# jkk-research/urban_road_filter

Hardware: AMD Instinct MI355X
Metric: scans/sec (64-ring x 2048-column cloud) (higher is better)
Workload: dtype f32+f64; 1 GPU; cfg3: batch of 1024 independent 64x2048 street sweeps per GPU, all three detectors + blind_spots, reference default parameters with ROI x,y widened to +-200 m, inputs resident in HBM (SoA x/y/z); scans_per_gpu=1024

## Files before the change

urban_road_filter_amd/csrc/urf_api.hip:

```cpp
#include <hip/hip_runtime.h>

#include <cmath>
#include <cstdio>
#include <cstdlib>
#include <cstring>
#include <ctime>
#include <string>
#include <vector>
#if defined(__SSE2__)
#include <emmintrin.h>
#include <xmmintrin.h>
#endif

#include "urf.h"
#ifdef URF_ENABLE_TEST_HOOKS
#include "urf_test_hooks.h"
#endif
#include "urf_internal.hpp"
#include "urf_kernels.hpp"
#include "urf_front.hpp"

#define URF_ASYNC_SLOTS 4
static_assert(URF_ASYNC_SLOTS == URF_MAX_IN_FLIGHT, "include/urf.h documents the number of sweeps in flight");

template <class T, bool Host = false>
struct lazy_buf {
    T* p = nullptr;
    size_t cap = 0;
    lazy_buf() = default;
    lazy_buf(const lazy_buf&) = delete;
    lazy_buf& operator=(const lazy_buf&) = delete;
    ~lazy_buf() { release(); }
    void release()
    {
        if (p)
            (void)(Host ? hipHostFree(p) : hipFree(p));
        p = nullptr;
        cap = 0;
    }
};

#define URF_SCRATCH_SCANS(X)                                                                                                     \
    X(rx, sstride) X(ry, sstride) X(rz, sstride) X(rec, sstride)                                                                 \
    X(sr, sstride) X(sz, sstride) X(sslot, sstride) X(ssrt16, sstride) X(ssrt, sstride) X(wsg, sstride)                          \
    X(big_r, sstride) X(big_z, sstride) X(big_i, sstride)                                                                        \
    X(tile_roi, max_tiles) X(roi_bits, max_tiles * (URF_TILE / 64)) X(troff, max_tiles * (URF_MAX_CHANNELS + 1))                 \
    X(tsoff, max_tiles * (URF_MAX_SECTORS + 1)) X(tmaxs, max_tiles * URF_MAX_CHANNELS)                                           \
    X(rpre, URF_MAX_CHANNELS * (max_tiles + 1)) X(rstart, URF_MAX_CHANNELS * max_tiles)                                          \
    X(angle, URF_MAX_CHANNELS) X(ring_thr, URF_MAX_CHANNELS * 4) X(ring_lut, URF_LUT_CELLS) X(ring_cnt, URF_MAX_CHANNELS)        \
    X(ring_off, URF_MAX_CHANNELS + 1)                                                                                            \
    X(sec_cnt, URF_MAX_SECTORS) X(sec_run, URF_MAX_SECTORS) X(sec_off, URF_MAX_SECTORS + 1) X(star_hit, URF_MAX_SECTORS)         \
    X(star_first, URF_MAX_SECTORS) X(star_list_mid, URF_MAX_SECTORS) X(star_list_big, URF_MAX_SECTORS)                           \
    X(star_list_runs, URF_MAX_SECTORS) X(tie_list, URF_MAX_SECTORS) X(tie_post, URF_MAX_SECTORS)                                 \
    X(table_upto, 1) X(table_redo, 1) X(redo_list, 1) X(table_cause, 1)                                                          \
    X(nan_mask, 4) X(nan_list, 2 * URF_MAX_CHANNELS) X(vis, URF_MAX_CHANNELS)                                                    \
    X(maxdist, URF_MAX_CHANNELS) X(quad, 4)                                                                                      \
    X(curb_cnt, URF_MAX_CHANNELS) X(curb_az, URF_MAX_CHANNELS * URF_CURB_LIST)                                                   \
    X(sufmin, URF_MAX_CHANNELS * URF_DEG_CELLS) X(premax, URF_MAX_CHANNELS * URF_DEG_CELLS)                                      \
    X(stop_f, URF_DEG_CELLS) X(stop_b, URF_DEG_CELLS)                                                                            \
    X(win, URF_MAX_CHANNELS * URF_DEG_CELLS)                                                                                     \
    X(info, 1)                                                                                                                   \
    X(front_ok, 1) X(front_pres, max_tiles * 64) X(front_maxs, max_tiles * 64) X(front_lane_ring, 64)                            \
    X(front_ring_lane, URF_MAX_CHANNELS) X(front_cand, front_cand_cap) X(front_all, front_cand_cap) X(front_ncand, 1)             \
    X(front_list, 1) X(front_st, URF_FRONT_ST_WORDS)
#define URF_SCRATCH_SLOTS(X) X(star_count, 8) X(ring_hint, 1)
#define URF_SCRATCH_CAPTURE(X) X(valpha, sstride) X(seckey, sstride) X(ringkey, sstride) X(rd2, sstride) X(caz, sstride)
#define URF_SCRATCH_ROW_MAJOR(X) X(tx, sstride) X(ty, sstride) X(tz, sstride) X(rows_v, 64) X(rows_ok, 1)
enum urf_scratch_group { URF_SCR_ALWAYS, URF_SCR_CAPTURE, URF_SCR_ROW_MAJOR };

struct __attribute__((visibility("hidden"))) urf_policy {
    uint32_t* flags = nullptr;
    uint64_t epoch = 1;
    bool speculate = true, use_hint = true;
    bool slot_lists = false, slot_nan = false, slot_ties = false;
    int front_mode = 1;
    uint32_t front_tpb = 0;
    bool want_ring_sorted = false;
    bool front_direct = false, front_off = false;
    bool front_rows = false, rows_oom = false, rows_used = false;
    uint32_t rows_probation = 0;

    template <class T>
    void set(T& field, T value)
    {
        if (field != value) {
            field = value;
            epoch++;
        }
    }
    void forget_front()
    {
        set(front_direct, false);
        set(front_off, false);
        flags[URF_FLAG_FRONT_HANDED_BACK] = flags[URF_FLAG_FRONT_ALL_HANDED_BACK] = 0;
    }
    int fold(urf_ctx* c, hipStream_t st);
    void probation_sweep() { lapse(front_rows); }
    void probation_batch(const urf_kargs& a) { lapse(a.front && front_mode != 2 && a.n_scans < URF_FRONT_MIN_SCANS); }
    void lapse(bool counts)
    {
        if (counts && !rows_used && rows_probation && --rows_probation == 0)
            epoch++;
    }
    bool on_redo(int status)
    {
        switch (status) {
        case URF_STATUS_REDO_TABLE: set(speculate, false); return true;
        case URF_STATUS_REDO_HINT: set(use_hint, false); return true;
        case URF_STATUS_REDO_LISTS: set(slot_lists, true); return true;
        case URF_STATUS_REDO_NAN: set(slot_nan, true); return true;
        case URF_STATUS_REDO_TIES: set(slot_ties, true); return true;
        }
        return false;
    }
    void plan(urf_kargs& a, const urf_dev_params& dp, bool slot, bool general_only) const
    {
        a.table_lookahead = speculate ? URF_TABLE_LOOKAHEAD : 0u;
        a.table_hint = (speculate && use_hint) ? 1u : 0u;
        a.optimistic = slot ? ((speculate ? URF_OPT_NO_REPAIR : 0u) | (slot_lists ? 0u : URF_OPT_NO_LISTS) | (slot_nan ? 0u : URF_OPT_NO_NAN) |
                               (slot_ties ? 0u : URF_OPT_NO_TIES)) : 0u;
        const unsigned L = (unsigned)dp.p.channels;
        const bool lasers = L == 64u || L == 32u || L == 16u;
        a.front_lsh = L == 16u ? 4u : (L == 32u ? 5u : 6u);
        const bool shape = front_mode != 0 && !front_off && !general_only && !want_ring_sorted && a.capture == 0 &&
                           lasers && dp.p.curbPoints == 5 && a.tiles <= URF_FRONT_MAX_TILES;
        const bool small_ok = front_rows && (rows_used || rows_probation > 0) && (L == 64u || front_mode == 2);
        a.front = (shape && (slot ? small_ok : (front_mode == 2 || small_ok || a.n_scans >= (L == 64u ? URF_FRONT_MIN_SCANS : (L == 32u ? URF_FRONT_MIN_SCANS_32 : URF_FRONT_MIN_SCANS_16))))) ? 1u : 0u;
        a.front_sight = (shape && !a.front && !front_rows && !rows_oom && (L == 64u || front_mode == 2)) ? 1u : 0u;
        a.front_tpb = front_tpb ? front_tpb : (a.n_scans >= URF_FRONT_TPB_SCANS ? URF_FRONT_TPB_LARGE : (a.n_scans >= 16u ? URF_FRONT_TPB_SMALL : 1u));
        a.front_lists = (a.front && !front_direct && !slot) ? 1u : 0u;
        a.front_rows = (a.front && front_rows) ? 1u : 0u;
    }
};

enum urf_last_kind { URF_LAST_NONE, URF_LAST_SOA, URF_LAST_PC2, URF_LAST_SWEEP };
struct urf_last_call {
    int kind = URF_LAST_NONE;
    uint32_t scans = 0;
    urf_kargs a;
    urf_dev_params dp;
    uint32_t row = 0;
    uint64_t gen = 0;
};

struct urf_ctx {
    int device = 0;
    uint32_t max_points = 0, max_batch = 0;
    uint32_t max_tiles = 0;
    uint32_t sstride = 0;
    uint32_t debug_flags = 0;
    unsigned n_cus = 256;
    hipStream_t own_stream = nullptr;
    hipStream_t stream = nullptr;
    urf_params params;
    urf_dev_params dp;
    urf_kargs k;
    std::vector<void*> allocs;
    lazy_buf<float> sx, sy, sz;
    struct slot_t {
        lazy_buf<uint8_t, true> h_in;
        lazy_buf<uint8_t> d_raw;
        lazy_buf<uint8_t, true> h_labels;
        lazy_buf<uint8_t> d_labels;
        lazy_buf<urf_scan_info, true> h_info;
        hipEvent_t ev_done = nullptr;
        hipGraph_t graph = nullptr;
        hipGraphExec_t exec = nullptr;
        uint64_t key[3] = { 0, 0, 0 };
        urf_kargs cap_a;
        urf_dev_params cap_dp;
        bool pending = false, used = false;
        uint64_t gen = 0;
        uint32_t n_points = 0, ticket = 0;
        uint32_t point_step = 0, off_x = 0, off_y = 0, off_z = 0;
        bool planes = false;
    } slots[URF_ASYNC_SLOTS];
    bool streams_made = false;
    urf_policy pol;
    uint32_t n_rerun = 0;
    hipStream_t row_stream[URF_ASYNC_SLOTS] = { nullptr, nullptr, nullptr, nullptr };
    hipEvent_t ev_main = nullptr;
    uint64_t main_seq = 1;
    uint64_t row_seen[URF_ASYNC_SLOTS] = { 0, 0, 0, 0 };
    uint64_t row_gen[URF_ASYNC_SLOTS] = { 0, 0, 0, 0 };
    uint32_t next_ticket = 0;
    lazy_buf<unsigned long long> ord_keys;
    lazy_buf<uint32_t> ord_pos;
    lazy_buf<uint32_t> ord_cls;
    lazy_buf<uint32_t> ord_lists;
    lazy_buf<float> mk_d;
    lazy_buf<uint32_t> mk_pos;
    lazy_buf<uint8_t> mk_red;
    lazy_buf<float> mk_out;
    lazy_buf<int32_t> mk_ghost;
    uint32_t* compact_cnt = nullptr;
    lazy_buf<urf_u32x4> cl_tiles;
    lazy_buf<uint32_t> cl_lists;
    float* d_newY = nullptr;
    urf_beam* d_beams = nullptr;
    uint32_t beams_cap = 0;
    int capture = 0;
    bool timing = false;
    std::vector<std::vector<hipEvent_t>> timing_events;
    size_t timing_used = 0;
    uint32_t* offsets_copy = nullptr;
    hipStream_t side_stream = nullptr;
    hipEvent_t ev_fork = nullptr, ev_join = nullptr;
    urf_last_call last;
    std::string last_error;
    double ht[8] = { 0, 0, 0, 0, 0, 0, 0, 0 };
    bool ht_on = false;
};

#define URF_HIP(ctx, call)                                                              \
    do {                                                                                \
        hipError_t e_ = (call);                                                         \
        if (e_ != hipSuccess) {                                                         \
            (ctx)->last_error = std::string(#call) + ": " + hipGetErrorString(e_);      \
            return e_ == hipErrorOutOfMemory ? URF_ERR_OOM : URF_ERR_HIP;               \
        }                                                                               \
    } while (0)

template <class T>
static int dev_alloc(urf_ctx* c, T** p, size_t count)
{
    void* v = nullptr;
    URF_HIP(c, hipMalloc(&v, (count ? count : 1) * sizeof(T)));
    c->allocs.push_back(v);
    *p = (T*)v;
    return URF_OK;
}

template <class T, bool Host>
static int grow(urf_ctx* c, lazy_buf<T, Host>& b, size_t count, hipStream_t st = nullptr)
{
    if (count <= b.cap)
        return URF_OK;
    if (st)
        URF_HIP(c, hipStreamSynchronize(st));
    b.release();
    void* v = nullptr;
    URF_HIP(c, Host ? hipHostMalloc(&v, count * sizeof(T), hipHostMallocDefault) : hipMalloc(&v, count * sizeof(T)));
    b.p = (T*)v;
    b.cap = count;
    return URF_OK;
}
// ... 123 lines not shown
extern "C" int urf_create(urf_ctx** out, int device_id, uint32_t max_points, uint32_t max_batch)
{
    if (!out || max_points == 0 || max_batch == 0)
        return URF_ERR_INVALID_ARG;
    *out = nullptr;
    const unsigned long long max_tiles = ((unsigned long long)max_points + URF_TILE - 1) / URF_TILE;
    const unsigned long long sstride = max_tiles * URF_TILE + URF_SCAN_PAD;
    if (max_tiles > URF_MAX_TILES || sstride * max_batch >= (1ull << 32))
        return URF_ERR_CAPACITY;
    int ndev = 0;
    if (hipGetDeviceCount(&ndev) != hipSuccess || ndev <= 0 || device_id < 0 || device_id >= ndev)
        return URF_ERR_NO_DEVICE;
    urf_ctx* c = new urf_ctx();
    c->device = device_id;
    c->max_points = max_points;
    c->max_batch = max_batch;
    c->max_tiles = (uint32_t)max_tiles;
    c->sstride = (uint32_t)sstride;
    int rc = URF_OK;
    auto fail = [&](int code) {
        urf_destroy(c);
        return code;
    };
    if (hipSetDevice(device_id) != hipSuccess)
        return fail(URF_ERR_NO_DEVICE);
    if (hipStreamCreateWithFlags(&c->own_stream, hipStreamNonBlocking) != hipSuccess)
        return fail(URF_ERR_HIP);
    c->stream = c->own_stream;
    {
        hipDeviceProp_t prop;
        if (hipGetDeviceProperties(&prop, device_id) == hipSuccess && prop.multiProcessorCount > 0)
            c->n_cus = (unsigned)prop.multiProcessorCount;
    }
    urf_default_params(&c->params);
    std::memset(&c->k, 0, sizeof(c->k));
    std::memset(&c->last.a, 0, sizeof(c->last.a));
    urf_kargs& k = c->k;
    k.front_cand_cap = max_points / 8 > 4096 ? max_points / 8 : 4096;
    if ((rc = scratch_alloc(c, URF_SCR_ALWAYS)) != URF_OK || (rc = dev_alloc(c, &c->offsets_copy, (size_t)max_batch + 1)) != URF_OK ||
        (rc = dev_alloc(c, &c->compact_cnt, (size_t)max_batch * c->max_tiles * 4)) != URF_OK ||
        (rc = dev_alloc(c, &c->d_newY, (size_t)max_points)) != URF_OK || (rc = dev_alloc(c, &c->d_beams, (size_t)URF_MAX_SECTORS)) != URF_OK)
        return fail(rc);
    {
        urf_wu* tab = nullptr;
        const size_t nt = (size_t)max_points + 32;
        if ((rc = dev_alloc(c, &tab, nt)) != URF_OK)
            return fail(rc);
        hipLaunchKernelGGL(k_walk_table, dim3((unsigned)((nt + 255) / 256)), dim3(256), 0, c->stream, tab, (unsigned)nt);
        k.walk_tab = tab;
    }
    k.sstride = c->sstride;
    if (const char* e = std::getenv("URF_FRONT_TPB"))
        c->pol.front_tpb = (uint32_t)std::atoi(e) > 0 ? (uint32_t)std::atoi(e) : c->pol.front_tpb;
    {
        void* hp = nullptr;
        if (hipHostMalloc(&hp, URF_FLAG_WORDS * sizeof(uint32_t), hipHostMallocMapped) != hipSuccess)
            return fail(URF_ERR_HIP);
        c->pol.flags = (uint32_t*)hp;
        std::memset(hp, 0, URF_FLAG_WORDS * sizeof(uint32_t));
        if (hipMemset(k.ring_hint, 0, URF_ASYNC_SLOTS * sizeof(uint32_t)) != hipSuccess)
            return fail(URF_ERR_HIP);
        void* dp_ = nullptr;
        if (hipHostGetDevicePointer(&dp_, hp, 0) != hipSuccess)
            return fail(URF_ERR_HIP);
        k.flags = (uint32_t*)dp_;
    }
    {
        std::vector<float> newY(max_points);
        newY[0] = 0.0f;
        for (uint32_t j = 1; j < max_points; j++)
            newY[j] = (float)((double)newY[j - 1] + 0.0100);
        if (hipMemcpy(c->d_newY, newY.data(), newY.size() * sizeof(float), hipMemcpyHostToDevice) != hipSuccess)
            return fail(URF_ERR_HIP);
    }
    k.newY = c->d_newY;
    k.beams = c->d_beams;
    if ((rc = upload_params(c)) != URF_OK)
        return fail(rc);
    *out = c;
    return URF_OK;
}

extern "C" int urf_destroy(urf_ctx* c)
{
    if (!c)
        return URF_ERR_INVALID_ARG;
    (void)hipSetDevice(c->device);
    if (c->own_stream)
        (void)hipStreamSynchronize(c->own_stream);
    if (c->side_stream) {
        (void)hipStreamSynchronize(c->side_stream);
        (void)hipStreamDestroy(c->side_stream);
        (void)hipEventDestroy(c->ev_fork);
        (void)hipEventDestroy(c->ev_join);
    }
    for (hipStream_t st : c->row_stream)
        if (st)
            (void)hipStreamSynchronize(st);
    for (auto& set : c->timing_events)
        for (hipEvent_t e : set)
            (void)hipEventDestroy(e);
    for (void* p : c->allocs)
        (void)hipFree(p);
    if (c->pol.flags)
        (void)hipHostFree(c->pol.flags);
    for (auto& sl : c->slots) {
// ... 189 lines not shown
static int order_after_slots(urf_ctx* c)
{
    for (auto& sl : c->slots)
        if (sl.pending && sl.ev_done)
            URF_HIP(c, hipStreamWaitEvent(c->stream, sl.ev_done, 0));
    c->main_seq++;
    return URF_OK;
}
static int order_row_after_main(urf_ctx* c, uint32_t row, hipStream_t st)
{
    if (st == c->stream || c->row_seen[row] == c->main_seq)
        return URF_OK;
    if (!c->ev_main)
        URF_HIP(c, hipEventCreateWithFlags(&c->ev_main, hipEventDisableTiming));
    URF_HIP(c, hipEventRecord(c->ev_main, c->stream));
    URF_HIP(c, hipStreamWaitEvent(st, c->ev_main, 0));
    c->row_seen[row] = c->main_seq;
    return URF_OK;
}

struct urf_call {
    const float *x, *y, *z;
    const uint32_t* offsets;
    uint32_t n_per_scan, max_len, n_scans;
    uint8_t* labels;
    urf_scan_info* info;
    uint32_t row = 0;
    hipStream_t stream = nullptr;
    const urf_dev_params* dp = nullptr;
    int capture = -1;
    bool general_only = false;
};

static bool side_fork(urf_ctx* c, hipStream_t st)
{
    if (!c->side_stream) {
        hipStream_t s = nullptr;
        hipEvent_t f = nullptr, j = nullptr;
        if (hipStreamCreateWithFlags(&s, hipStreamNonBlocking) == hipSuccess && hipEventCreateWithFlags(&f, hipEventDisableTiming) == hipSuccess &&
            hipEventCreateWithFlags(&j, hipEventDisableTiming) == hipSuccess) {
            c->side_stream = s;
            c->ev_fork = f;
            c->ev_join = j;
        } else {
            if (f)
                (void)hipEventDestroy(f);
            if (s)
                (void)hipStreamDestroy(s);
        }
    }
    return c->side_stream && hipEventRecord(c->ev_fork, st) == hipSuccess && hipStreamWaitEvent(c->side_stream, c->ev_fork, 0) == hipSuccess;
}

static int run_pipeline(urf_ctx* c, const urf_call& call, urf_kargs& a_out, urf_dev_params& dp_out)
{
    if (!call.x || !call.y || !call.z || !call.labels)
        return URF_ERR_INVALID_ARG;
    const uint32_t n_scans = call.n_scans;
    if (n_scans == 0)
        return URF_OK;
    if (call.row + n_scans > c->max_batch || call.max_len > c->max_points)
        return URF_ERR_CAPACITY;
    URF_HIP(c, hipSetDevice(c->device));
    const bool slot = call.stream != nullptr;
    hipStream_t st = slot ? call.stream : c->stream;
    if (!slot) {
        int rc = order_after_slots(c);
        if (rc == URF_OK)
            rc = c->pol.fold(c, st);
        if (rc != URF_OK)
            return rc;
    }
    urf_kargs a = kargs_row(c, call.row);
    a.x = call.x;
    a.y = call.y;
    a.z = call.z;
    a.offsets = nullptr;
    if (call.offsets) {
        if (call.offsets != c->offsets_copy)
            URF_HIP(c, hipMemcpyAsync(c->offsets_copy, call.offsets, ((size_t)n_scans + 1) * sizeof(uint32_t), hipMemcpyDeviceToDevice, st));
        a.offsets = c->offsets_copy;
    }
    a.n_per_scan = call.n_per_scan;
    a.n_scans = n_scans;
    a.max_len = call.max_len;
    a.tiles = (call.max_len + URF_TILE - 1) / URF_TILE;
    if (a.tiles == 0)
        a.tiles = 1;
    a.sstride = c->sstride;
    a.capture = (uint32_t)(call.capture >= 0 ? call.capture : c->capture);
    a.labels = call.labels;
    if (a.capture != 1) {
        a.rd2 = nullptr;
        a.caz = nullptr;
    }
    const urf_dev_params dp = call.dp ? *call.dp : c->dp;
    const unsigned C = (unsigned)dp.p.channels, K = (unsigned)dp.p.sectors;
    const bool star = dp.p.star_shaped_method != 0;
    const dim3 g_tiles(a.tiles, n_scans), g_scan(n_scans);
    c->pol.plan(a, dp, slot, call.general_only);
    if (!slot)
        c->pol.probation_batch(a);

    std::vector<hipEvent_t>* ev = nullptr;
    if (c->timing) {
        if (c->timing_used == c->timing_events.size()) {
            c->timing_events.emplace_back(URF_NUM_KERNELS + 1);
            for (hipEvent_t& e : c->timing_events.back())
                URF_HIP(c, hipEventCreate(&e));
        }
        ev = &c->timing_events[c->timing_used++];
    }
    int stage = 0;
    auto mark = [&]() {
        if (ev)
            (void)hipEventRecord((*ev)[stage], st);
        stage++;
    };
    mark();
    if (a.front_rows)
        hipLaunchKernelGGL(k_rows_probe, g_scan, dim3(256), 0, st, a, dp);
    hipLaunchKernelGGL(k_ring_table, g_scan, dim3(URF_TABLE_THREADS), 0, st, a, dp);
    mark();
    if (a.front_rows)
        hipLaunchKernelGGL(k_transpose, g_tiles, dim3(256), 0, st, a);
    if (a.front) {
        const dim3 g_front((a.tiles + a.front_tpb - 1) / a.front_tpb, n_scans);
        if (a.front_lsh == 6u)
            hipLaunchKernelGGL(k_front, g_front, dim3(64), 0, st, a, dp);
        else if (a.front_lsh == 5u)
            hipLaunchKernelGGL(k_front32, g_front, dim3(64), 0, st, a, dp);
        else
            hipLaunchKernelGGL(k_front16, g_front, dim3(64), 0, st, a, dp);
    }
    if (a.front_lists) {
        hipLaunchKernelGGL(k_table_repair, g_scan, dim3(URF_TABLE_THREADS), 0, st, a, dp, 1u);
        hipLaunchKernelGGL(k_split_list, dim3(c->n_cus * 2), dim3(URF_TILE_THREADS), urf_split_lds_bytes(C, K, star), st, a, dp);
    } else {
        hipLaunchKernelGGL(k_split, g_tiles, dim3(URF_TILE_THREADS), urf_split_lds_bytes(C, K, star), st, a, dp);
    }
    if ((a.table_lookahead || a.front_rows) && !(a.optimistic & URF_OPT_NO_REPAIR)) {
        hipLaunchKernelGGL(k_table_repair, g_scan, dim3(URF_TABLE_THREADS), 0, st, a, dp, 0u);
        hipLaunchKernelGGL(k_split_repair, dim3(c->n_cus), dim3(URF_TILE_THREADS), urf_split_lds_bytes(C, K, star), st, a, dp);
    }
    mark();
    bool side = false, part1 = false;
    const size_t finish_lds = (size_t)a.tiles * 384 + 2 * URF_FINISH_CHUNK * sizeof(urf_u2);
    if (a.front && !ev && !slot && side_fork(c, st)) {
        hipLaunchKernelGGL(k_front_finish, g_scan, dim3(URF_FINISH_THREADS), finish_lds, c->side_stream, a, dp, 1u);
        part1 = true;
        side = hipEventRecord(c->ev_join, c->side_stream) == hipSuccess;
        if (!side)
            (void)hipStreamSynchronize(c->side_stream);
    }
    hipLaunchKernelGGL(k_index, g_scan, dim3(256), 0, st, a, dp);
    mark();
    const unsigned tie_grid = K * n_scans < c->n_cus * 4u ? K * n_scans : c->n_cus * 4u;
    const unsigned tie_grid_small = K * n_scans < c->n_cus * 16u ? K * n_scans : c->n_cus * 16u;
    if (star) {
        const dim3 g_sec(K, n_scans);
        hipLaunchKernelGGL(k_star_sort_small, g_sec, dim3(URF_STAR_THREADS), 0, st, a, dp);
        if (!(a.optimistic & URF_OPT_NO_LISTS)) {
            hipLaunchKernelGGL(k_star_sort_mid, dim3(c->n_cus * (URF_MID_WAVES * 256 / URF_STAR_MID_THREADS)), dim3(URF_STAR_MID_THREADS), 0, st,
                               a, dp);
            hipLaunchKernelGGL(k_star_sort_big, dim3(c->n_cus * 2), dim3(256), 0, st, a, dp);
            hipLaunchKernelGGL(k_star_sort_runs, dim3(c->n_cus * 20), dim3(URF_STAR_THREADS), 0, st, a, dp);
        }
        if (!(a.optimistic & URF_OPT_NO_TIES)) {
            hipLaunchKernelGGL((k_star_ties<false, URF_TIE_SMALL>), dim3(tie_grid_small), dim3(64), 0, st, a, dp);
            hipLaunchKernelGGL((k_star_ties<false, URF_TIE_CAP>), dim3(tie_grid), dim3(64), 0, st, a, dp);
        }
    }
    mark();
    if (star) {
        if (n_scans <= URF_WALK_FEW_SCANS)
            hipLaunchKernelGGL(k_star_walk_few, dim3((K + 63) / 64, n_scans), dim3(URF_WALK_FEW_THREADS), 0, st, a, dp);
        else
            hipLaunchKernelGGL(k_star_walk, dim3((K + 63) / 64, n_scans), dim3(64), 0, st, a, dp);
        if (!(a.optimistic & URF_OPT_NO_TIES)) {
            hipLaunchKernelGGL((k_star_ties<true, URF_TIE_SMALL>), dim3(tie_grid_small), dim3(64), 0, st, a, dp);
// ... 1002 lines not shown
```

urban_road_filter_amd/csrc/urf_front.hpp:

```cpp
#ifndef URF_FRONT_HPP
#define URF_FRONT_HPP

#define URF_FRONT_HPRE 8u
#ifndef URF_FRONT_HPOST
#define URF_FRONT_HPOST 8u
#endif
#define URF_FRONT_LANES 64u
#define URF_FRONT_STEPS (URF_TILE / URF_FRONT_LANES)
#define URF_FRONT_MIN_SCANS 192u
#define URF_FRONT_MIN_SCANS_32 0xffffffffu
#define URF_FRONT_MIN_SCANS_16 0xffffffffu
#define URF_FRONT_TPB_SMALL 2u
#define URF_FRONT_TPB_LARGE 4u
#define URF_FRONT_TPB_SCANS 512u
#define URF_FRONT_MAX_TILES 128u
#define URF_FRONT_RING_NONE 0x7fu
#define URF_FC_XZ 1u
#define URF_FC_ZZ 2u
#define URF_FC_EDGE_X 4u
#define URF_FC_EDGE_Z 8u
#ifndef URF_FRONT_NT
#define URF_FRONT_NT 0
#endif
#ifndef URF_FRONT_WAVES
#define URF_FRONT_WAVES 5
#endif

struct urf_front_thr {
    float y, z, below;
};
__device__ __forceinline__ urf_front_thr urf_front_load_thr(const urf_kargs& a, unsigned s, unsigned C, unsigned e, unsigned nR)
{
    urf_front_thr t;
    const bool valid = e < nR;
    const float4 tv = ((const float4*)a.ring_thr)[(size_t)s * C + (valid ? e : 0u)];
    const float bl = a.ring_thr[((size_t)s * C + ((valid && e) ? e - 1u : 0u)) * 4];
    t.y = valid ? tv.y : __builtin_inff();
    t.z = tv.z;
    t.below = e ? bl : __builtin_inff();
    return t;
}

__device__ __forceinline__ __amdgpu_buffer_rsrc_t urf_buf(const void* p, unsigned bytes)
{
    return __builtin_amdgcn_make_buffer_rsrc((void*)p, 0, (int)bytes, 0x00020000);
}
#define URF_OOB 0xffffffffu

__device__ __forceinline__ void urf_front_src(const urf_kargs& a, unsigned s, unsigned off, unsigned ok, const float*& gx, const float*& gy, const float*& gz)
{
    const bool rows = ok == URF_FRONT_ROWS;
    const size_t o = rows ? (size_t)urf_sbase(a, s) : (size_t)off;
    gx = (rows ? (const float*)a.tx : a.x) + o;
    gy = (rows ? (const float*)a.ty : a.y) + o;
    gz = (rows ? (const float*)a.tz : a.z) + o;
}

__global__ __launch_bounds__(256) void k_transpose(urf_kargs a)
{
    __shared__ float T[3][64 * 33];
    const unsigned s = blockIdx.y, t = blockIdx.x, tid = threadIdx.x;
    const unsigned lsh = a.front_lsh, L = 1u << lsh, wsh = 11u - lsh, W = 1u << wsh, RS = W + 1u;
    static_assert(URF_TILE == 2048u, "a tile's columns: 1 << (11 - lsh)");
    if (a.front_ok[s] != URF_FRONT_ROWS)
        return;
    unsigned off, len;
    urf_scan_range(a, s, off, len);
    const unsigned F = len >> lsh, f0 = t * W;
// ... 30 lines not shown
}

#define URF_FO_ADOPT 0x20000000u
#define URF_FO_NONE 0x40000000u
#define URF_FO_FAIL 0x80000000u
__device__ __noinline__ unsigned urf_front_open(const float* tab, unsigned nR, float interval, float x, float y, float z, unsigned sectors, float Kfi,
                                                unsigned E, unsigned econf)
{
    const urf_exact_key ek = urf_exact_keys_body(tab, nR, interval, x, y, z, sectors, Kfi);
    unsigned r = sectors ? ((ek.sector + 1u) & 0x7ffu) << 1 : 0u;
    if (ek.ring == URF_RING_NONE)
        r |= URF_FO_NONE;
    else if (x == 0.0f && y == 0.0f)
        r |= URF_FO_FAIL;
    else if (ek.ring == E)
        r |= 1u;
    else if (!econf)
        r |= 1u | URF_FO_ADOPT | (ek.ring << 12);
    else
        r |= URF_FO_FAIL;
    return r;
}

#define URF_FRONT_CBUF 256u
__device__ __forceinline__ void urf_front_flush(const urf_kargs& a, unsigned s, urf_u2* cbuf, unsigned& ncb, bool& overflow)
{
    if (ncb == 0u)
        return;
    urf_wave_lds_sync();
    unsigned base = 0;
    if (urf_lane() == 0u)
        base = atomicAdd(&a.front_ncand[s], ncb);
    base = (unsigned)__builtin_amdgcn_readfirstlane((int)base);
    for (unsigned j = urf_lane(); j < ncb; j += 64u) {
        if (base + j < a.front_cand_cap)
            a.front_cand[(size_t)s * a.front_cand_cap + base + j] = cbuf[j];
        else
            overflow = true;
    }
    urf_wave_lds_sync();
    ncb = 0;
}
__device__ __forceinline__ void urf_front_push(urf_u2* cbuf, unsigned& ncb, bool has, unsigned idx, unsigned what)
{
    const unsigned long long m = __ballot(has);
    if (has)
        cbuf[ncb + urf_popc_below(m)] = urf_u2{ idx, what };
    ncb += (unsigned)__popcll(m);
}

template <bool STAR, bool BEAM, unsigned L>
__device__ __forceinline__ void urf_front_body(const urf_kargs& a, const urf_dev_params& dp, urf_u2* cbuf)
{
    const unsigned s = blockIdx.y, b = blockIdx.x, lane = threadIdx.x;
    unsigned off, len;
    urf_scan_range(a, s, off, len);
    const unsigned TPB = a.front_tpb;
    const unsigned t_first = b * TPB;
    if (t_first * URF_TILE >= len)
        return;
    const unsigned ok = a.front_ok[s];
    if (ok == 0u)
        return;
    constexpr unsigned C = L;
    constexpr unsigned STEPS = URF_TILE / L;
    static_assert(L == 64u || L == 32u || L == 16u, "a firing fills the wave, half of it or a quarter");
    const unsigned K = (unsigned)dp.p.sectors;
    const unsigned nf = (len + L - 1u) / L;
    const unsigned F0 = t_first * STEPS;
    const unsigned F1 = F0 + TPB * STEPS < nf ? F0 + TPB * STEPS : nf;
    const unsigned Fs = F0 > URF_FRONT_HPRE ? F0 - URF_FRONT_HPRE : 0u;
    const unsigned Fe = F1 + URF_FRONT_HPOST < nf ? F1 + URF_FRONT_HPOST : nf;
    const bool from_start = Fs == 0u;
    const bool to_end = Fe == nf;
    static_assert(URF_FRONT_HPRE % 4u == 0u && STEPS % 4u == 0u, "the march runs in groups of four firings");
    const unsigned sb = urf_sbase(a, s);
    const float *gx, *gy, *gz;
    urf_front_src(a, s, off, ok, gx, gy, gz);
    const __amdgpu_buffer_rsrc_t brec = urf_buf(a.rec + sb, len * 4u);
    const __amdgpu_buffer_rsrc_t bsr = urf_buf(a.sr + sb, a.tiles * URF_TILE * 4u), bsz = urf_buf(a.sz + sb, a.tiles * URF_TILE * 4u);
    const __amdgpu_buffer_rsrc_t bss = urf_buf(a.sslot + sb, a.tiles * URF_TILE * 2u);
    const unsigned nR = a.info[s].n_rings;
    const unsigned upto_v = a.table_upto[s];
    const unsigned upto = ok == URF_FRONT_ROWS ? 0u : (nR < C ? upto_v : 0xffffffffu);
    const float* const tab = a.angle + (size_t)s * dp.p.channels;
    const float curbH = dp.p.curbHeight;
    const bool use_x = dp.p.x_zero_method != 0, use_z = dp.p.z_zero_method != 0;

    unsigned E = lane;
    bool econf = false;
    urf_front_thr th = urf_front_load_thr(a, s, C, E, nR);
    bool failed = false, overflow = false;
    unsigned long long failed_m = 0;
    unsigned ncb = 0;

    float w0 = 0.f, w1 = 0.f, w2 = 0.f, w3 = 0.f, w4 = 0.f, w5 = 0.f, w6 = 0.f, w7 = 0.f, w8 = 0.f, w9 = 0.f, w10 = 0.f;
    unsigned fwA = 0, fwB = 0, fwC = 0;
    unsigned wc = 0;
    unsigned tot = 0, nin = 0;
    double maxs = 0.0;
    unsigned pw = 0;
    unsigned troi = 0, tstar = 0;
    int stepkey_v = (int)URF_SEC_NONE, stepcnt_v = 0;
    int stepkey_w = (int)URF_SEC_NONE, stepcnt_w = 0;

    auto step = [&](auto ph, const unsigned f, const float x, const float y, const float z) {
        constexpr unsigned PH = decltype(ph)::value;
        const unsigned stp = f % STEPS;
        const unsigned i = f * L + lane;
        const bool roi = (L == 64u || lane < L) && i < len && urf_in_roi(dp.p, x, y, z);
        const unsigned long long roim = __ballot(roi);
// ... 215 lines not shown
        py[j] = gy[o];
        pz[j] = gz[o];
    };
#pragma unroll
    for (unsigned j = 0; j < 4; j++)
        ld(j, Fs + j);
    for (unsigned f = Fs; f < F0; f += 4) {
#pragma unroll
        for (unsigned j = 0; j < 4; j++) {
            step(std::integral_constant<unsigned, 0u>{}, f + j, px[j], py[j], pz[j]);
            ld(j, f + j + 4u);
        }
    }
    for (unsigned f = F0; f < F1; f += 4) {
#pragma unroll
        for (unsigned j = 0; j < 4; j++) {
            if (f + j < F1)
                step(std::integral_constant<unsigned, 1u>{}, f + j, px[j], py[j], pz[j]);
            ld(j, f + j + 4u);
        }
        if (L != 64u && (((f + 4u) & 31u) == 0u || f + 4u >= F1))
            pres_end(f >> 5);
        if (((f + 4u) % STEPS) == 0u || f + 4u >= F1) {
            tile_end(f / STEPS);
            if (failed_m != 0ull || __ballot(failed | overflow) != 0ull) {
                a.front_ok[s] = 0u;
                if (ok == URF_FRONT_ROWS)
                    a.table_redo[s] = 1u;
                return;
            }
        }
    }
    for (unsigned f = F1; f < Fe; f += 4) {
#pragma unroll
        for (unsigned j = 0; j < 4; j++) {
            if (f + j < Fe)
                step(std::integral_constant<unsigned, 2u>{}, f + j, px[j], py[j], pz[j]);
            ld(j, f + j + 4u);
        }
    }
    if (!to_end) {
        const unsigned fr[5] = { fwA >> 16, fwB & 0xffffu, fwB >> 16, fwC & 0xffffu, fwC >> 16 };
#pragma unroll
        for (unsigned e = 0; e < 5; e++) {
            const unsigned back = 4u - e;
            const bool in = tot > back && tot - back <= nin;
            const unsigned what = (use_z ? URF_FC_EDGE_Z : 0u) | ((use_x && e >= 2u) ? URF_FC_EDGE_X : 0u);
            if (ncb > URF_FRONT_CBUF - 64u)
                urf_front_flush(a, s, cbuf, ncb, overflow);
            urf_front_push(cbuf, ncb, in && what != 0u, (fr[e] + Fs) * L + lane, what);
        }
    }
    urf_front_flush(a, s, cbuf, ncb, overflow);
    a.front_maxs[((size_t)s * a.tiles + b) * 64u + lane] = (unsigned long long)__double_as_longlong(maxs);
    if (econf) {
        const unsigned o1 = atomicCAS(&a.front_lane_ring[(size_t)s * 64u + lane], 0xffffffffu, E);
        const unsigned o2 = atomicCAS(&a.front_ring_lane[(size_t)s * C + E], 0xffffffffu, lane);
        failed = failed | (o1 != 0xffffffffu && o1 != E) | (o2 != 0xffffffffu && o2 != lane);
    }
    if (failed_m != 0ull || __ballot(failed | overflow) != 0ull) {
        a.front_ok[s] = 0u;
        if (ok == URF_FRONT_ROWS)
            a.table_redo[s] = 1u;
    }
}

template <unsigned L>
__device__ __forceinline__ void urf_front_kernel(const urf_kargs& a, const urf_dev_params& dp, urf_u2* cbuf)
{
    if (!dp.p.star_shaped_method)
        urf_front_body<false, false, L>(a, dp, cbuf);
    else if (!dp.p.starbeam_filter)
        urf_front_body<true, false, L>(a, dp, cbuf);
    else
        urf_front_body<true, true, L>(a, dp, cbuf);
}
#define URF_FRONT_KERNEL(name, L)                                                                                                             \
    __global__ __launch_bounds__(64) __attribute__((amdgpu_waves_per_eu(URF_FRONT_WAVES, URF_FRONT_WAVES))) void name(urf_kargs a, urf_dev_params dp) \
    {                                                                                                                                         \
        __shared__ urf_u2 cbuf[URF_FRONT_CBUF];                                                                                               \
        urf_front_kernel<L>(a, dp, cbuf);                                                                                                     \
    }
URF_FRONT_KERNEL(k_front, 64u)
URF_FRONT_KERNEL(k_front32, 32u)
URF_FRONT_KERNEL(k_front16, 16u)

#define URF_FRONT_ST_WORDS 72u
#define URF_FINISH_CHUNK 768u
#ifndef URF_FINISH_THREADS
#define URF_FINISH_THREADS 256
#endif
struct urf_finish_shared {
    unsigned n[64];
    unsigned ring[64];
    unsigned ncurb[URF_FRONT_LANES];
    int q[4];
    unsigned n_pend;
    unsigned nx, nz;
    unsigned qsum[URF_FINISH_THREADS / 64][64];
};

__device__ __forceinline__ unsigned urf_front_prev(const unsigned* P, unsigned lsh, unsigned l, unsigned f)
{
    unsigned t = f >> 5;
    unsigned w = P[(t << lsh) + l] & ((1u << (f & 31u)) - 1u);
    while (w == 0u) {
        if (t == 0u)
// ... 49 lines not shown
    unsigned m_from = 0;
    if (part != 2u) {
    const urf_u2* const cand = a.front_cand + (size_t)s * a.front_cand_cap;
    const unsigned nc_raw = a.front_ncand[s];
    const unsigned nc = nc_raw < a.front_cand_cap ? nc_raw : a.front_cand_cap;
    for (unsigned k = tid; k < npt * L; k += URF_FINISH_THREADS)
        P[k] = a.front_pres[(size_t)s * a.tiles * 64u + k];
    if (tid < URF_FRONT_LANES)
        S.ncurb[tid] = 0;
    if (tid < 64)
        S.ring[tid] = a.front_lane_ring[(size_t)s * 64u + tid];
    if (tid == 0) {
        st[70] = 0;
        S.q[0] = (int)urf_fbits(0.f);
        S.q[1] = (int)urf_fbits(180.f);
        S.q[2] = (int)urf_fbits(180.f);
        S.q[3] = (int)urf_fbits(360.f);
        S.n_pend = 0;
    }
    __syncthreads();
    {
        constexpr unsigned NP = URF_FINISH_THREADS / 64u;
        const unsigned l = tid & 63u, prt = tid >> 6;
        const unsigned nt = l < L ? npt : 0u;
        const unsigned tq = (nt + NP - 1u) / NP, ta = prt * tq < nt ? prt * tq : nt, tb = ta + tq < nt ? ta + tq : nt;
        unsigned run = 0;
        for (unsigned t = ta; t < tb; t++)
            run += (unsigned)__popc(P[(t << lsh) + l]);
        S.qsum[prt][l] = run;
        __syncthreads();
        unsigned add = 0, all = 0;
        for (unsigned p = 0; p < NP; p++) {
            add += p < prt ? S.qsum[p][l] : 0u;
            all += S.qsum[p][l];
        }
        for (unsigned t = ta; t < tb; t++) {
            B[(t << lsh) + l] = (uint16_t)add;
            add += (unsigned)__popc(P[(t << lsh) + l]);
        }
        if (prt == 0)
            S.n[l] = all;
    }
    if (tid < C)
        a.ring_cnt[(size_t)s * C + tid] = 0;
    __syncthreads();
    if (tid < 64) {
        const unsigned r = S.ring[tid], n = r != 0xffffffffu ? S.n[tid] : 0u;
        unsigned tot = n;
        for (int o = 32; o > 0; o >>= 1)
            tot += __shfl_xor(tot, o);
        if (r != 0xffffffffu) {
            a.ring_cnt[(size_t)s * C + r] = n;
            unsigned long long m = 0;
            const unsigned nblk = (ntiles + a.front_tpb - 1u) / a.front_tpb;
            for (unsigned b0 = 0; b0 < nblk; b0 += 8u) {
                unsigned long long v[8];
#pragma unroll
                for (unsigned b = 0; b < 8; b++)
                    v[b] = a.front_maxs[((size_t)s * a.tiles + (b0 + b < nblk ? b0 + b : b0)) * 64u + tid];
#pragma unroll
                for (unsigned b = 0; b < 8; b++)
                    m = v[b] > m ? v[b] : m;
            }
            a.maxdist[(size_t)s * C + r] = (float)__builtin_sqrt(__longlong_as_double((long long)m));
            a.vis[(size_t)s * C + r] = urf_vis{ __builtin_inff(), -__builtin_inff() };
            if (r == 10u)
                st[70] = n;
        }
        if (tid == 0)
            st[69] = tot;
    }
    constexpr unsigned CH = URF_FINISH_CHUNK;
    for (unsigned c0 = 0; c0 < nc; c0 += CH) {
        const unsigned cn = nc - c0 < CH ? nc - c0 : CH;
        if (tid == 0) {
            S.nx = 0;
            S.nz = 0;
        }
        __syncthreads();
        for (unsigned e = tid; e < cn; e += URF_FINISH_THREADS) {
            const urf_u2 cd = cand[c0 + e];
            if (cd.y & (URF_FC_XZ | URF_FC_EDGE_X))
                chunk[atomicAdd(&S.nx, 1u)] = cd;
            if (cd.y & (URF_FC_ZZ | URF_FC_EDGE_Z))
                chunk[2u * CH - 1u - atomicAdd(&S.nz, 1u)] = cd;
        }
        __syncthreads();
        const unsigned nx = S.nx, nz = S.nz;
        if (dp.p.x_zero_method)
            for (unsigned e = tid; e < nx; e += URF_FINISH_THREADS) {
                const urf_u2 cd = chunk[e];
                const unsigned idx = cd.x, l = idx & lm, f = idx >> lsh;
                const unsigned n = S.n[l];
                const unsigned p = (unsigned)B[((f >> 5) << lsh) + l] + (unsigned)__popc(P[((f >> 5) << lsh) + l] & ((1u << (f & 31u)) - 1u));
                if (!(p >= 7u && p + 3u < n))
                    continue;
                unsigned fj = urf_front_prev(P, lsh, l, f);
                fj = urf_front_prev(P, lsh, l, fj);
                unsigned f3 = urf_front_next(P, lsh, npt, l, f);
                f3 = urf_front_next(P, lsh, npt, l, f3);
                f3 = urf_front_next(P, lsh, npt, l, f3);
                const unsigned ij = (fj << lsh) + l, i3 = (f3 << lsh) + l;
                const float pz = gz[idx], xj = gx[ij], yj = gy[ij], zj = gz[ij], x3 = gx[i3], y3 = gy[i3], z3 = gz[i3];
                const float nyj = a.newY[p - 2u], ny2 = a.newY[p], ny3 = a.newY[p + 3u];
                bool heights = true;
                if (cd.y & URF_FC_EDGE_X)
                    heights = (__builtin_fabsf(zj - pz) >= dp.p.curbHeight || __builtin_fabsf(z3 - pz) >= dp.p.curbHeight) &&
                              (double)__builtin_fabsf(zj - z3) >= 0.05;
                if (heights && urf_x_zero_angle_vals(nyj, ny2, ny3, dp.p.angleFilter1, dp.x_angle_thr, xj, yj, x3, y3, zj, pz, z3))
                    passed(idx, 2u);
            }
        if (dp.p.z_zero_method)
// ... 359 lines not shown
```

urban_road_filter_amd/csrc/urf_internal.hpp:

```cpp
#ifndef URF_INTERNAL_HPP
#define URF_INTERNAL_HPP

#include <cstddef>
#include <cstdint>

#include "urf.h"

#define URF_MAX_CHANNELS    128
#define URF_MAX_SECTORS     1022
#define URF_MAX_CURB_POINTS 30
#define URF_LUT_UMAX        4.0f
#define URF_LUT_SCALE       512.0f
#define URF_LUT_CELLS       4100
#define URF_DEG_CELLS       361

#define URF_TILE            2048
#ifndef URF_TILE_THREADS
#define URF_TILE_THREADS    512
#endif
#define URF_TILE_GROUPS     (URF_TILE / 64)
#define URF_MAX_TILES       4096
#define URF_SCAN_PAD        512
#define URF_SLOT_NONE       0xFFFFu
#define URF_SLOT_OFF        0x8000u
#define URF_TABLE_LOOKAHEAD 8192

#define URF_REC_SRC_MASK    0x7FFu
#define URF_REC_FLAG_SHIFT  11
#define URF_REC_AZ_SHIFT    14
#define URF_REC_AZ_UNKNOWN  0x3FFFFu
#define URF_REC_AZ_SCALE    (262143.0f / 360.0f)
#define URF_REC_AZ_STEP     (360.0f / 262143.0f)
#define URF_REC_AZ_QERR     9.0e-4f
#define URF_OPT_NO_REPAIR 1u
#define URF_OPT_NO_LISTS 2u
#define URF_OPT_NO_NAN 4u
#define URF_OPT_NO_TIES 8u
#define URF_STATUS_REDO_TABLE 0x7f000001
#define URF_STATUS_REDO_LISTS 0x7f000002
#define URF_STATUS_REDO_NAN 0x7f000003
#define URF_STATUS_REDO_HINT 0x7f000004
#define URF_STATUS_REDO_TIES 0x7f000005
enum urf_flag {
    URF_FLAG_LOOKAHEAD_FAILED = 0,
    URF_FLAG_HINT_FAILED = 1,
    URF_FLAG_FRONT_HANDED_BACK = 2,
    URF_FLAG_FRONT_ALL_HANDED_BACK = 3,
    URF_FLAG_ROWS_SIGHTED = 4,
    URF_FLAG_ROWS_TAKEN = 6,
    URF_FLAG_WORDS = 8
};
#define URF_TIE_FLAG 0x80000000u
#define URF_TIE_NEXT 0x40000000u
#define URF_TIE_DONE 0x20000000u
#define URF_TIE_POST 0x10000000u
#define URF_TIE_INDEX 0x00ffffffu
#define URF_TIE_CAP 2048u
// ... 1 lines not shown
#define URF_RING_NONE       0xFFu
#define URF_SEC_NONE        0x3FFu

int urf_validate_params(const urf_params* p);

struct urf_beam {
    int32_t yx;
    float   d;
    float   o;
};

struct urf_dev_params {
    urf_params p;
    float    slope_param;
    float    Kfi;
    float    sector_margin;
    float    fwd_limit;
    float    bwd_limit;
    float    inv_cp;
    float    x_angle_thr;
    float    z_angle_thr;
    uint32_t sec_keybits;
    uint32_t ring_keybits;
    uint32_t exp_flags;
};

#define URF_RUNS_FLAG 0x40000000u
struct urf_sec_run { uint32_t a0, c0, a1, nruns; };

struct alignas(8) urf_sg { float slp, g; };
struct alignas(8) urf_wu { float w, u; };

struct alignas(8) urf_vis { float f_hi, b_lo; };

struct alignas(8) urf_u2 { uint32_t x, y; };

struct urf_win { float hi, lo; };

struct urf_kargs {
    const float* x;
    const float* y;
    const float* z;
    const uint32_t* offsets;
    uint32_t n_per_scan;
    uint32_t n_scans;
    uint32_t max_len;
    uint32_t tiles;
    uint32_t sstride;
    uint32_t table_lookahead;
    uint32_t table_hint;
    uint32_t optimistic;
    uint32_t capture;
    uint32_t  front;
    uint32_t  front_tpb;
    uint32_t  front_cand_cap;
    uint32_t  front_pad_;
    uint8_t* labels;
    urf_scan_info* info;
    float*    valpha;
    uint16_t* seckey;
    uint8_t*  ringkey;
    float*    caz;
    float*    rx;
    float*    ry;
    float*    rz;
    uint32_t* rec;
    float*    rd2;
    float*    sr;
    float*    sz;
    uint16_t* sslot;
    uint16_t* ssrt16;
    uint32_t* ssrt;
    urf_sg*   wsg;
    const urf_wu* walk_tab;
    uint32_t* tile_roi;
    uint16_t* troff;
    uint16_t* tsoff;
    unsigned long long* tmaxs;
    uint32_t* rpre;
    uint16_t* rstart;
    float*    angle;
    uint8_t*  ring_lut;
    float*    ring_thr;
    uint32_t* ring_cnt;
    uint32_t* ring_off;
    uint32_t* sec_cnt;
    urf_sec_run* sec_run;
    uint32_t* sec_off;
    int32_t*  star_hit;
    uint32_t* star_first;
    uint32_t* star_list_mid;
    uint32_t* star_list_big;
    uint32_t* star_list_runs;
    uint32_t* tie_list;
    uint32_t* tie_post;
    uint32_t* star_count;
    uint32_t* table_upto;
    uint32_t* table_redo;
    uint32_t* redo_list;
    uint32_t* table_cause;
    uint32_t* ring_hint;
    uint32_t* flags;
    float*    big_r;
    float*    big_z;
    uint32_t* big_i;
    uint32_t* nan_mask;
    uint32_t* nan_list;
    urf_vis*  vis;
    float*    maxdist;
    float*    quad;
    uint32_t* curb_cnt;
    float*    curb_az;
    float*    sufmin;
    float*    premax;
    int16_t*  stop_f;
    int16_t*  stop_b;
    unsigned long long* roi_bits;
    urf_win*  win;
    const float*    newY;
    const urf_beam* beams;
    uint32_t* front_ok;
    uint32_t* front_pres;
    unsigned long long* front_maxs;
    uint32_t* front_lane_ring;
    uint32_t* front_ring_lane;
    urf_u2*   front_cand;
    urf_u2*   front_all;
    uint32_t* front_ncand;
    uint32_t* front_st;
    uint32_t* front_list;
    uint32_t  front_lsh;
    uint32_t  front_lists;
    uint32_t  front_rows;
    uint32_t  front_sight;
    float*    rows_v;
    uint32_t* rows_ok;
    float*    tx;
    float*    ty;
    float*    tz;
};
#define URF_FRONT_ROWS 2u

#endif
```

Before: 470,200 scans/s.

## Launch front kernel from a host-built block plan with variable tile runs

```diff
diff --git a/urban_road_filter_amd/csrc/urf_api.hip b/urban_road_filter_amd/csrc/urf_api.hip
--- a/urban_road_filter_amd/csrc/urf_api.hip
+++ b/urban_road_filter_amd/csrc/urf_api.hip
@@ -75,6 +75,7 @@
     bool slot_lists = false, slot_nan = false, slot_ties = false;
     int front_mode = 1;
     uint32_t front_tpb = 0;
+    std::vector<uint32_t> front_lens;
     bool want_ring_sorted = false;
     bool front_direct = false, front_off = false;
     bool front_rows = false, rows_oom = false, rows_used = false;
@@ -112,6 +113,12 @@
         case URF_STATUS_REDO_TIES: set(slot_ties, true); return true;
         }
         return false;
+    }
+    std::vector<uint32_t> block_tiles(uint32_t n_scans) const
+    {
+        if (!front_lens.empty())
+            return front_lens;
+        return { front_tpb ? front_tpb : (n_scans >= 512u ? 4u : (n_scans >= 16u ? 2u : 1u)) };
     }
     void plan(urf_kargs& a, const urf_dev_params& dp, bool slot, bool general_only) const
     {
@@ -127,7 +134,6 @@
         const bool small_ok = front_rows && (rows_used || rows_probation > 0) && (L == 64u || front_mode == 2);
         a.front = (shape && (slot ? small_ok : (front_mode == 2 || small_ok || a.n_scans >= (L == 64u ? URF_FRONT_MIN_SCANS : (L == 32u ? URF_FRONT_MIN_SCANS_32 : URF_FRONT_MIN_SCANS_16))))) ? 1u : 0u;
         a.front_sight = (shape && !a.front && !front_rows && !rows_oom && (L == 64u || front_mode == 2)) ? 1u : 0u;
-        a.front_tpb = front_tpb ? front_tpb : (a.n_scans >= URF_FRONT_TPB_SCANS ? URF_FRONT_TPB_LARGE : (a.n_scans >= 16u ? URF_FRONT_TPB_SMALL : 1u));
         a.front_lists = (a.front && !front_direct && !slot) ? 1u : 0u;
         a.front_rows = (a.front && front_rows) ? 1u : 0u;
     }
@@ -192,6 +198,11 @@
     lazy_buf<uint32_t> mk_pos;
     lazy_buf<uint8_t> mk_red;
     lazy_buf<float> mk_out;
+    lazy_buf<unsigned long long> plan_dev;
+    lazy_buf<unsigned long long, true> plan_host;
+    uint32_t plan_scans = 0, plan_tiles = 0, plan_blocks = 0;
+    std::vector<uint32_t> plan_lens;
+    unsigned long long* plan_one = nullptr;
     lazy_buf<int32_t> mk_ghost;
     uint32_t* compact_cnt = nullptr;
     lazy_buf<urf_u32x4> cl_tiles;
@@ -421,6 +432,28 @@
     k.sstride = c->sstride;
     if (const char* e = std::getenv("URF_FRONT_TPB"))
         c->pol.front_tpb = (uint32_t)std::atoi(e) > 0 ? (uint32_t)std::atoi(e) : c->pol.front_tpb;
+    if (const char* e = std::getenv("URF_FRONT_PLAN"))
+        for (const char* q = e; *q;) {
+            char* end = nullptr;
+            const unsigned long v = std::strtoul(q, &end, 10);
+            if (end == q)
+                break;
+            c->pol.front_lens.push_back((uint32_t)(v < 1ul ? 1ul : (v > URF_FRONT_MAX_TILES ? (unsigned long)URF_FRONT_MAX_TILES : v)));
+            q = *end == ',' ? end + 1 : end;
+        }
+    {
+        const uint32_t nt = c->max_tiles < URF_FRONT_MAX_TILES ? c->max_tiles : URF_FRONT_MAX_TILES, one = 1u;
+        std::vector<urf_u2> plan;
+        std::vector<unsigned long long> starts;
+        urf_front_plan_build(1, nt, &one, 1, plan, starts);
+        std::vector<unsigned long long> both(starts);
+        for (const urf_u2& d : plan)
+            both.push_back((unsigned long long)d.x | ((unsigned long long)d.y << 32));
+        if ((rc = dev_alloc(c, &c->plan_one, both.size())) != URF_OK)
+            return fail(rc);
+        if (hipMemcpy(c->plan_one, both.data(), both.size() * sizeof(unsigned long long), hipMemcpyHostToDevice) != hipSuccess)
+            return fail(URF_ERR_HIP);
+    }
     {
         void* hp = nullptr;
         if (hipHostMalloc(&hp, URF_FLAG_WORDS * sizeof(uint32_t), hipHostMallocMapped) != hipSuccess)
@@ -716,6 +749,34 @@
     return c->side_stream && hipEventRecord(c->ev_fork, st) == hipSuccess && hipStreamWaitEvent(c->side_stream, c->ev_fork, 0) == hipSuccess;
 }
 
+static int front_plan_batch(urf_ctx* c, urf_kargs& a, hipStream_t st)
+{
+    std::vector<uint32_t> lens = c->pol.block_tiles(a.n_scans);
+    if (!c->plan_dev.p || c->plan_scans != a.n_scans || c->plan_tiles != a.tiles || c->plan_lens != lens) {
+        std::vector<urf_u2> plan;
+        std::vector<unsigned long long> starts;
+        urf_front_plan_build(a.n_scans, a.tiles, lens.data(), (uint32_t)lens.size(), plan, starts);
+        const size_t n = starts.size() + plan.size();
+        URF_HIP(c, hipStreamSynchronize(st));
+        c->plan_scans = 0;
+        int rc;
+        if ((rc = grow(c, c->plan_dev, n)) != URF_OK || (rc = grow(c, c->plan_host, n)) != URF_OK)
+            return rc;
+        std::memcpy(c->plan_host.p, starts.data(), starts.size() * sizeof(unsigned long long));
+        static_assert(sizeof(urf_u2) == sizeof(unsigned long long), "a descriptor is one 8-byte word");
+        std::memcpy(c->plan_host.p + starts.size(), plan.data(), plan.size() * sizeof(urf_u2));
+        URF_HIP(c, hipMemcpyAsync(c->plan_dev.p, c->plan_host.p, n * sizeof(unsigned long long), hipMemcpyHostToDevice, st));
+        c->plan_scans = a.n_scans;
+        c->plan_tiles = a.tiles;
+        c->plan_blocks = (uint32_t)plan.size();
+        c->plan_lens.swap(lens);
+    }
+    a.front_starts = c->plan_dev.p;
+    a.front_plan = (const urf_u2*)(c->plan_dev.p + 2 * (size_t)a.n_scans);
+    a.front_blocks = c->plan_blocks;
+    return URF_OK;
+}
+
 static int run_pipeline(urf_ctx* c, const urf_call& call, urf_kargs& a_out, urf_dev_params& dp_out)
 {
     if (!call.x || !call.y || !call.z || !call.labels)
@@ -765,6 +826,16 @@
     c->pol.plan(a, dp, slot, call.general_only);
     if (!slot)
         c->pol.probation_batch(a);
+    a.front_blocks = 0;
+    if (a.front && slot) {
+        a.front_starts = c->plan_one;
+        a.front_plan = (const urf_u2*)(c->plan_one + 2);
+        a.front_blocks = a.tiles;
+    } else if (a.front) {
+        const int rc = front_plan_batch(c, a, st);
+        if (rc != URF_OK)
+            return rc;
+    }
 
     std::vector<hipEvent_t>* ev = nullptr;
     if (c->timing) {
@@ -789,7 +860,7 @@
     if (a.front_rows)
         hipLaunchKernelGGL(k_transpose, g_tiles, dim3(256), 0, st, a);
     if (a.front) {
-        const dim3 g_front((a.tiles + a.front_tpb - 1) / a.front_tpb, n_scans);
+        const dim3 g_front(a.front_blocks);
         if (a.front_lsh == 6u)
             hipLaunchKernelGGL(k_front, g_front, dim3(64), 0, st, a, dp);
         else if (a.front_lsh == 5u)
diff --git a/urban_road_filter_amd/csrc/urf_front.hpp b/urban_road_filter_amd/csrc/urf_front.hpp
--- a/urban_road_filter_amd/csrc/urf_front.hpp
+++ b/urban_road_filter_amd/csrc/urf_front.hpp
@@ -10,10 +10,7 @@
 #define URF_FRONT_MIN_SCANS 192u
 #define URF_FRONT_MIN_SCANS_32 0xffffffffu
 #define URF_FRONT_MIN_SCANS_16 0xffffffffu
-#define URF_FRONT_TPB_SMALL 2u
-#define URF_FRONT_TPB_LARGE 4u
-#define URF_FRONT_TPB_SCANS 512u
-#define URF_FRONT_MAX_TILES 128u
+static_assert(URF_FRONT_MAX_TILES * (URF_TILE / 16u) + URF_FRONT_HPRE + URF_FRONT_HPOST <= 0xffffu, "firings of a block of k_front: 16 bits");
 #define URF_FRONT_RING_NONE 0x7fu
 #define URF_FC_XZ 1u
 #define URF_FC_ZZ 2u
@@ -150,11 +147,10 @@
 template <bool STAR, bool BEAM, unsigned L>
 __device__ __forceinline__ void urf_front_body(const urf_kargs& a, const urf_dev_params& dp, urf_u2* cbuf)
 {
-    const unsigned s = blockIdx.y, b = blockIdx.x, lane = threadIdx.x;
+    const urf_u2 blk = a.front_plan[blockIdx.x];
+    const unsigned s = blk.x, t_first = blk.y & 0xffffu, TPB = blk.y >> 16, lane = threadIdx.x;
     unsigned off, len;
     urf_scan_range(a, s, off, len);
-    const unsigned TPB = a.front_tpb;
-    const unsigned t_first = b * TPB;
     if (t_first * URF_TILE >= len)
         return;
     const unsigned ok = a.front_ok[s];
@@ -476,7 +472,7 @@
         }
     }
     urf_front_flush(a, s, cbuf, ncb, overflow);
-    a.front_maxs[((size_t)s * a.tiles + b) * 64u + lane] = (unsigned long long)__double_as_longlong(maxs);
+    a.front_maxs[((size_t)s * a.tiles + t_first) * 64u + lane] = (unsigned long long)__double_as_longlong(maxs);
     if (econf) {
         const unsigned o1 = atomicCAS(&a.front_lane_ring[(size_t)s * 64u + lane], 0xffffffffu, E);
         const unsigned o2 = atomicCAS(&a.front_ring_lane[(size_t)s * C + E], 0xffffffffu, lane);
@@ -632,12 +628,23 @@
         if (r != 0xffffffffu) {
             a.ring_cnt[(size_t)s * C + r] = n;
             unsigned long long m = 0;
-            const unsigned nblk = (ntiles + a.front_tpb - 1u) / a.front_tpb;
-            for (unsigned b0 = 0; b0 < nblk; b0 += 8u) {
+            unsigned long long b0 = a.front_starts[2u * s], b1 = a.front_starts[2u * s + 1u];
+            b0 &= ntiles < 64u ? (1ull << ntiles) - 1ull : ~0ull;
+            b1 &= ntiles <= 64u ? 0ull : (ntiles < 128u ? (1ull << (ntiles - 64u)) - 1ull : ~0ull);
+            while ((b0 | b1) != 0ull) {
                 unsigned long long v[8];
-#pragma unroll
-                for (unsigned b = 0; b < 8; b++)
-                    v[b] = a.front_maxs[((size_t)s * a.tiles + (b0 + b < nblk ? b0 + b : b0)) * 64u + tid];
+                unsigned t = 0;
+#pragma unroll
+                for (unsigned b = 0; b < 8; b++) {
+                    if (b0 != 0ull) {
+                        t = (unsigned)__ffsll((long long)b0) - 1u;
+                        b0 &= b0 - 1ull;
+                    } else if (b1 != 0ull) {
+                        t = 64u + (unsigned)__ffsll((long long)b1) - 1u;
+                        b1 &= b1 - 1ull;
+                    }
+                    v[b] = a.front_maxs[((size_t)s * a.tiles + t) * 64u + tid];
+                }
 #pragma unroll
                 for (unsigned b = 0; b < 8; b++)
                     m = v[b] > m ? v[b] : m;
diff --git a/urban_road_filter_amd/csrc/urf_internal.hpp b/urban_road_filter_amd/csrc/urf_internal.hpp
--- a/urban_road_filter_amd/csrc/urf_internal.hpp
+++ b/urban_road_filter_amd/csrc/urf_internal.hpp
@@ -3,6 +3,7 @@
 
 #include <cstddef>
 #include <cstdint>
+#include <vector>
 
 #include "urf.h"
 
@@ -110,7 +111,7 @@
     uint32_t optimistic;
     uint32_t capture;
     uint32_t  front;
-    uint32_t  front_tpb;
+    uint32_t  front_blocks;
     uint32_t  front_cand_cap;
     uint32_t  front_pad_;
     uint8_t* labels;
@@ -186,6 +187,8 @@
     urf_u2*   front_all;
     uint32_t* front_ncand;
     uint32_t* front_st;
+    const urf_u2* front_plan;
+    const unsigned long long* front_starts;
     uint32_t* front_list;
     uint32_t  front_lsh;
     uint32_t  front_lists;
@@ -198,5 +201,35 @@
     float*    tz;
 };
 #define URF_FRONT_ROWS 2u
+#define URF_FRONT_MAX_TILES 128u
+
+inline void urf_front_plan_build(uint32_t n_scans, uint32_t tiles, const uint32_t* lens, uint32_t n_lens, std::vector<urf_u2>& plan,
+                                 std::vector<unsigned long long>& starts)
+{
+    std::vector<uint32_t> cut;
+    for (uint32_t t = 0, k = 0; t < tiles; k++) {
+        uint32_t n = (lens && n_lens) ? lens[k % n_lens] : 1u;
+        n = n < 1u ? 1u : (n > URF_FRONT_MAX_TILES ? URF_FRONT_MAX_TILES : n);
+        n = n < tiles - t ? n : tiles - t;
+        cut.push_back(n);
+        t += n;
+    }
+    uint32_t first[URF_FRONT_MAX_TILES + 2] = { 0 };
+    for (uint32_t n : cut)
+        first[n - 1] += n_scans;
+    for (uint32_t n = URF_FRONT_MAX_TILES; n-- > 0;)
+        first[n] += first[n + 1];
+    plan.assign((size_t)cut.size() * n_scans, urf_u2{ 0, 0 });
+    starts.assign((size_t)2 * n_scans, 0ull);
+    for (uint32_t s = 0; s < n_scans; s++) {
+        uint32_t t = 0;
+        for (uint32_t n : cut) {
+            plan[first[n]++] = urf_u2{ s, t | (n << 16) };
+            if (t < 2u * 64u)
+                starts[(size_t)2 * s + (t >> 6)] |= 1ull << (t & 63u);
+            t += n;
+        }
+    }
+}
 
 #endif
```

Result: no change. 471,600 scans/s (median of 4 runs) (+0.3%).
